# QY-H00/attention-interpolation-diffusion

Measured on AMD Instinct MI355X. Metric: interpolation-frames/sec (50-step), higher is better.
Workload: dtype bf16

## Files before the change

attention-interpolation-diffusion_amd/csrc/aid_gemm.hip:

```cpp
#include "aid_common.hpp"
#include "aid_kernels.hpp"

#include <stdlib.h>
#include <string.h>

#include <type_traits>

namespace aid {

struct TileCoord {
    int p, batch, m0, n0;
};

template <int NB, int MB>
__device__ __forceinline__ void mfma_fence(f32x16 (&acc)[NB][MB]) {
#pragma unroll
    for (int i = 0; i < NB; ++i)
#pragma unroll
        for (int j = 0; j < MB; ++j) asm volatile("" : "+v"(acc[i][j]));
    asm volatile("s_nop 15\n\ts_nop 3" ::: "memory");
#pragma unroll
    for (int i = 0; i < NB; ++i)
#pragma unroll
        for (int j = 0; j < MB; ++j) asm volatile("" : "+v"(acc[i][j]));
// ... 562 lines not shown
                            asm volatile("" : "+v"(t));
                            v[e] = fmaf(lc1[e], t, lr1[im]);
                        }
                    }
#pragma unroll
                    for (int e = 0; e < 4; ++e) v[e] = fmaf(v[e], P.scale, bv[e]);
                    *reinterpret_cast<T4*>(Cs + (wm + im * 32 + l31) * CLD + nl) = cvt4<T>(v);
                }
            }
        __syncthreads();
        const bool vec_ok = (P.ldc % 8 == 0) && ((reinterpret_cast<uintptr_t>(C) & 15) == 0);
        constexpr int CPRW = BN / 8;
#pragma unroll
        for (int it = 0; it < (BM * CPRW) / NTHR; ++it) {
            const int id = tid + it * NTHR;
            const int row = id / CPRW, ch = (id % CPRW) * 8;
            const int m = m0 + row, n = n0 + ch;
            if (m >= P.m || n >= P.n) continue;
            T8 v = *reinterpret_cast<const T8*>(Cs + row * CLD + ch);
            T* dst = C + (int64_t)m * P.ldc + n;
            const T* res = R ? R + (int64_t)m * P.ldc + n : nullptr;
            if (vec_ok && n + 8 <= P.n) {
                if (res) {
                    const bool rvec = (reinterpret_cast<uintptr_t>(R) & 15) == 0;
                    T8 r;
                    if (rvec) {
                        r = *reinterpret_cast<const T8*>(res);
                    } else {
#pragma unroll
                        for (int e = 0; e < 8; ++e) r[e] = res[e];
                    }
                    const f32x8 a = up8<T>(v), b = up8<T>(r);
                    v = cvt8<T>(a + b);
                }
                *reinterpret_cast<T8*>(dst) = v;
            } else {
                const int n4 = (P.n + 3) & ~3;
#pragma unroll
                for (int e = 0; e < 8; ++e) {
                    if (n + e < P.n) dst[e] = res ? (T)((float)v[e] + (float)res[e]) : v[e];
                    else if (n + e < n4) dst[e] = (T)0.f;
                }
            }
        }
    }
};

template <typename T>
struct PingPong : Engine<T, 256, 256, 64, 2, 2, 4> {
    typedef Engine<T, 256, 256, 64, 2, 2, 4> Base;
    typedef typename Vec<T>::v8 T8;
    static constexpr int HALF = 128 * 128;
    static constexpr int STG = 4 * HALF;
    static constexpr size_t SMEM = Base::SMEM;
    using Base::smem; using Base::tid; using Base::lane; using Base::wave; using Base::wm; using Base::wn;
    using Base::l31; using Base::hi; using Base::aoff; using Base::boff; using Base::ax; using Base::bx;
    using Base::acc;
    typedef __amdgpu_buffer_rsrc_t Rsrc;
    int wr;
    Rsrc ra, rb;
    int avo[4], bvo[4];

    static __device__ __forceinline__ int swz(int r) { return (r >> 1) & 7; }

    __device__ __forceinline__ void init(char* smem_) {
        smem = smem_;
        tid = threadIdx.x;
        lane = tid & 63;
        wave = __builtin_amdgcn_readfirstlane(tid >> 6);
        wr = wave >> 2;
        wm = wr * 128;
        wn = (wave & 3) * 64;
        l31 = lane & 31;
        hi = lane >> 5;
#pragma unroll
        for (int e = 0; e < 2; ++e) {
            const int lr = wr * 64 + e * 32 + l31;
            aoff[e] = lr * 128;
            ax[e] = hi ^ swz(lr);
        }
        const int lb = (wave & 3) * 32 + l31;
        boff[0] = 2 * HALF + lb * 128;
        bx[0] = hi ^ swz(lb);
    }

    __device__ __forceinline__ void set_tile(const GemmDesc& P, const T* A, const T* B, int m0, int n0) {
#pragma unroll
        for (int h = 0; h < 2; ++h)
#pragma unroll
            for (int j = 0; j < 2; ++j) {
                const int lrow = 8 * (2 * wave + j) + (lane >> 3);
                const int c = (lane & 7) ^ swz(lrow);
                const int row_a = (lrow >> 6) * 128 + h * 64 + (lrow & 63);
                const int row_b = (lrow >> 5) * 64 + h * 32 + (lrow & 31);
                avo[h * 2 + j] = min(row_a, P.m - 1 - m0) * (P.lda * 2) + c * 16;
                bvo[h * 2 + j] = min(row_b, P.n - 1 - n0) * (P.ldb * 2) + c * 16;
            }
        ra = __builtin_amdgcn_make_buffer_rsrc(const_cast<T*>(A + (int64_t)m0 * P.lda), 0, 0x7fffffff, 0x00020000);
        rb = __builtin_amdgcn_make_buffer_rsrc(const_cast<T*>(B + (int64_t)n0 * P.ldb), 0, 0x7fffffff, 0x00020000);
    }

    __device__ __forceinline__ void set_tile_lr(int m, int n, int lda, int ldb, const T* A, const T* B, int m0, int n0) {
        int ln = lane;
        asm volatile("" : "+v"(ln));
#pragma unroll
        for (int h = 0; h < 2; ++h)
#pragma unroll
            for (int j = 0; j < 2; ++j) {
                const int lrow = 8 * (2 * wave + j) + (ln >> 3);
                const int c = (ln & 7) ^ swz(lrow);
                const int row_a = (lrow >> 6) * 128 + h * 64 + (lrow & 63);
                const int row_b = (lrow >> 5) * 64 + h * 32 + (lrow & 31);
                avo[h * 2 + j] = min(row_a, m - 1 - m0) * (lda * 2) + c * 16;
                bvo[h * 2 + j] = min(row_b, n - 1 - n0) * (ldb * 2) + c * 16;
            }
        ra = __builtin_amdgcn_make_buffer_rsrc(const_cast<T*>(A + (int64_t)m0 * lda), 0, 0x7fffffff, 0x00020000);
        rb = __builtin_amdgcn_make_buffer_rsrc(const_cast<T*>(B + (int64_t)n0 * ldb), 0, 0x7fffffff, 0x00020000);
    }

    static __device__ __forceinline__ float mulg(float a, float g) {
        float t = a * g;
        asm volatile("" : "+v"(t));
        return t;
    }
    __device__ __forceinline__ void scale_rows(const float* __restrict__ gain, int side, int m0, int n0, int M, int N) {
        mfma_fence(acc);
        const bool bym = side == 1;
        const int lim = bym ? M : N;
        float gm[4], gn[2][16];
#pragma unroll
        for (int im = 0; im < 4; ++im) {
            const float g = gain[min(m0 + wm + 32 * im + l31, lim - 1)];
            gm[im] = bym ? g : 1.f;
        }
#pragma unroll
        for (int in = 0; in < 2; ++in)
#pragma unroll
            for (int r = 0; r < 16; ++r) {
                const float g = gain[min(n0 + wn + 32 * in + hi * 4 + 8 * (r >> 2) + (r & 3), lim - 1)];
                gn[in][r] = bym ? 1.f : g;
            }
#pragma unroll
        for (int in = 0; in < 2; ++in)
#pragma unroll
            for (int im = 0; im < 4; ++im)
#pragma unroll
                for (int r = 0; r < 16; ++r) acc[in][im][r] = mulg(mulg(acc[in][im][r], gm[im]), gn[in][r]);
    }

    template <int Q>
    __device__ __forceinline__ void dma_one(int parity, int k0, int j) {
        constexpr bool IS_A = Q >= 2;
        constexpr int H = Q & 1;
        char* dst = smem + parity * STG + (IS_A ? 0 : 2 * HALF) + H * HALF + wave * 2048 + j * 1024;
        __builtin_amdgcn_raw_ptr_buffer_load_lds(IS_A ? ra : rb, (__attribute__((address_space(3))) void*)dst, 16,
                                                 IS_A ? avo[H * 2 + j] : bvo[H * 2 + j], k0 * 2, 0, 0);
    }

    static constexpr int E = 6;
    template <int S>
    __device__ __forceinline__ void issue_first(int kb, int nk) {
        if ((S >> 2) < nk) {
            dma_one<(S & 3)>((S >> 2) & 1, (kb + (S >> 2)) * 64, 0);
            dma_one<(S & 3)>((S >> 2) & 1, (kb + (S >> 2)) * 64, 1);
        }
        if constexpr (S + 1 < E) issue_first<S + 1>(kb, nk);
    }
    template <int P>
    __device__ __forceinline__ void issue(int kt, int kb, int nk, int i) {
        constexpr int S0 = 2 * P + E;
        const int s = S0 + (i >> 1);
        const int t = kt + (s >> 2);
        if (t < nk) {
            if ((S0 & 3) == 2) {
                if (i < 2) dma_one<2>(t & 1, (kb + t) * 64, i & 1);
                else       dma_one<3>(t & 1, (kb + t) * 64, i & 1);
            } else {
                if (i < 2) dma_one<0>(t & 1, (kb + t) * 64, i & 1);
                else       dma_one<1>(t & 1, (kb + t) * 64, i & 1);
            }
        }
    }
    template <int P>
    __device__ __forceinline__ void retire(int kt, int nk) {
        constexpr int NEWEST = 2 * P + E - 1;
        constexpr int NEED = P == 0 ? 3 : 6;
        static_assert(NEWEST >= NEED, "lead too short");
        if (kt + (NEWEST >> 2) < nk) wait_vmcnt<2 * (NEWEST - NEED)>();
        else                         wait_vmcnt<0>();
    }

    __device__ __forceinline__ void read_a(T8 (&fa)[2][4], const char* st, int h) {
#pragma unroll
        for (int e = 0; e < 2; ++e)
#pragma unroll
            for (int ks = 0; ks < 4; ++ks)
                fa[e][ks] = *reinterpret_cast<const T8*>(st + h * HALF + aoff[e] + (((2 * ks) ^ ax[e]) << 4));
    }
    __device__ __forceinline__ void read_b(T8 (&fb)[2][4], const char* st) {
#pragma unroll
        for (int j = 0; j < 2; ++j)
#pragma unroll
            for (int ks = 0; ks < 4; ++ks)
                fb[j][ks] = *reinterpret_cast<const T8*>(st + boff[0] + j * HALF + (((2 * ks) ^ bx[0]) << 4));
    }
    template <int P, bool DMA = true, bool PRIO = false>
    __device__ __forceinline__ void half(const T8 (&fb)[2][4], const T8 (&fa)[2][4], int kt, int kb, int nk) {
        if (PRIO) __builtin_amdgcn_s_setprio(1);
#pragma unroll
        for (int i = 0; i < 16; ++i) {
            const int ks = i >> 2, in = (i >> 1) & 1, e = i & 1;
            acc[in][2 * P + e] = mfma32(fb[in][ks], fa[e][ks], acc[in][2 * P + e]);
            if (DMA && (i == 2 || i == 5 || i == 8 || i == 11)) {
                __builtin_amdgcn_sched_barrier(0);
                issue<P>(kt, kb, nk, (i - 2) / 3);
                __builtin_amdgcn_sched_barrier(0);
            }
        }
        if (PRIO) __builtin_amdgcn_s_setprio(0);
    }
    static __device__ __forceinline__ void slot() {
        __builtin_amdgcn_sched_barrier(0);
        __builtin_amdgcn_s_barrier();
        __builtin_amdgcn_sched_barrier(0);
    }

    template <int Q>
    __device__ __forceinline__ void dma_half(int t, int kb) {
        dma_one<Q>(t & 1, (kb + t) * 64, 0);
        dma_one<Q>(t & 1, (kb + t) * 64, 1);
    }
    template <bool PRIO>
    __device__ __forceinline__ void mac_rd(int kb, int ke) {
        const int nk = ke - kb;
        dma_half<0>(0, kb); dma_half<1>(0, kb); dma_half<2>(0, kb); dma_half<3>(0, kb);
        if (nk > 1) { dma_half<0>(1, kb); dma_half<1>(1, kb); wait_vmcnt<6>(); }
        else        wait_vmcnt<2>();
        slot();
        if (wr == 1) slot();
        T8 fa[2][4], fb[2][4];
        auto body = [&](int kt, auto more1_t, auto more2_t) __attribute__((always_inline)) {
            constexpr bool M1 = decltype(more1_t)::value, M2 = decltype(more2_t)::value;
            const char* st = smem + (kt & 1) * STG;
            read_b(fb, st);
            read_a(fa, st, 0);
            if (M1) { dma_half<2>(kt + 1, kb); dma_half<3>(kt + 1, kb); }
            if (M1) asm volatile("s_waitcnt vmcnt(8) lgkmcnt(0)" ::: "memory");
            else    asm volatile("s_waitcnt vmcnt(0) lgkmcnt(0)" ::: "memory");
            slot();
            half<0, false, PRIO>(fb, fa, kt, kb, nk);
            slot();
            read_a(fa, st, 1);
            if (M2) { dma_half<0>(kt + 2, kb); dma_half<1>(kt + 2, kb); }
            if (M2)      asm volatile("s_waitcnt vmcnt(6) lgkmcnt(0)" ::: "memory");
            else if (M1) asm volatile("s_waitcnt vmcnt(2) lgkmcnt(0)" ::: "memory");
            else         asm volatile("s_waitcnt vmcnt(0) lgkmcnt(0)" ::: "memory");
            slot();
            half<1, false, PRIO>(fb, fa, kt, kb, nk);
            slot();
        };
        const std::true_type Y{};
        const std::false_type N{};
        int kt = 0;
        for (; kt + 2 < nk; ++kt) body(kt, Y, Y);
        if (kt + 1 < nk) { body(kt, Y, N); ++kt; }
        if (kt < nk) body(kt, N, N);
        if (wr == 0) slot();
        wait_vmcnt<0>();
        __syncthreads();
    }

    __device__ __forceinline__ void mac(int kb, int ke) {
        const int nk = ke - kb;
        issue_first<0>(kb, nk);
        if (nk >= 2) wait_vmcnt<2 * (E - 3)>();
        else         wait_vmcnt<0>();
        slot();
        if (wr == 1) slot();
        T8 fa[2][4], fb[2][4];
        for (int kt = 0; kt < nk; ++kt) {
            const char* st = smem + (kt & 1) * STG;
            read_b(fb, st);
            read_a(fa, st, 0);
            retire<0>(kt, nk);
            slot();
            half<0>(fb, fa, kt, kb, nk);
            slot();
            read_a(fa, st, 1);
            retire<1>(kt, nk);
            slot();
            half<1>(fb, fa, kt, kb, nk);
            slot();
        }
        if (wr == 0) slot();
        wait_vmcnt<0>();
        __syncthreads();
    }
};

constexpr int PP_SMALL_NS = 4;
static_assert(Engine<bf16, 128, 128, 64, PP_SMALL_NS, 2, 4>::SMEM <= PingPong<bf16>::SMEM, "small tiles use the big tile's LDS");


template <typename T>
struct PingPongX : PingPong<T> {
    typedef PingPong<T> PP;
    typedef typename Vec<T>::v8 T8;
    typedef typename Vec<T>::v4 T4;
    static constexpr int BMX = 288, XR = 32;
    static constexpr int HALF = PP::HALF;
    static constexpr int STGX = 4 * HALF + XR * 128;
    static constexpr int CLD = 256 + 8;
    static constexpr size_t LNS = (size_t)(BMX + 256) * 2 * sizeof(float);
    static constexpr size_t SMEMX = (size_t)BMX * CLD * 2 + LNS > (size_t)2 * STGX ? (size_t)BMX * CLD * 2 + LNS : (size_t)2 * STGX;
    static_assert(SMEMX <= 160 * 1024, "one workgroup per CU");
    using PP::smem; using PP::tid; using PP::lane; using PP::wave; using PP::wm; using PP::wn; using PP::wr;
    using PP::l31; using PP::hi; using PP::aoff; using PP::boff; using PP::ax; using PP::bx; using PP::acc;
    using PP::ra; using PP::rb; using PP::avo; using PP::bvo;
    f32x16 accx;
    int xoff, xx, xvo;

    __device__ __forceinline__ void init(char* smem_) {
        PP::init(smem_);
        xoff = 4 * HALF + l31 * 128;
        xx = hi ^ PP::swz(l31);
    }
    __device__ __forceinline__ void set_tile(const GemmDesc& P, const T* A, const T* B, int m0, int n0) {
        PP::set_tile(P, A, B, m0, n0);
        const int lrow = 8 * (wave & 3) + (lane >> 3);
        const int c = (lane & 7) ^ PP::swz(lrow);
        xvo = min(256 + lrow, P.m - 1 - m0) * (P.lda * 2) + c * 16;
    }
    __device__ __forceinline__ void zero_acc() {
        PP::zero_acc();
#pragma unroll
        for (int r = 0; r < 16; ++r) accx[r] = 0.f;
    }
    __device__ __forceinline__ void xdma_half(const int Q, int t, int kb) {
        const bool IS_A = Q >= 2;
        const int H = Q & 1;
#pragma unroll
        for (int j = 0; j < 2; ++j) {
            char* dst = smem + (t & 1) * STGX + (IS_A ? 0 : 2 * HALF) + H * HALF + wave * 2048 + j * 1024;
            __builtin_amdgcn_raw_ptr_buffer_load_lds(IS_A ? ra : rb, (__attribute__((address_space(3))) void*)dst, 16,
                                                     IS_A ? avo[H * 2 + j] : bvo[H * 2 + j], (kb + t) * 128, 0, 0);
        }
    }
    __device__ __forceinline__ void dma_strip(int t, int kb) {
        char* dst = smem + (t & 1) * STGX + 4 * HALF + wave * 1024;
        __builtin_amdgcn_raw_ptr_buffer_load_lds(ra, (__attribute__((address_space(3))) void*)dst, 16, xvo, (kb + t) * 128, 0, 0);
    }
    __device__ __forceinline__ void read_x(T8 (&fx)[4], const char* st) {
#pragma unroll
        for (int ks = 0; ks < 4; ++ks) fx[ks] = *reinterpret_cast<const T8*>(st + xoff + (((2 * ks) ^ xx) << 4));
    }
    template <int N>
    __device__ __forceinline__ void wait_rd(bool xw) {
        if (xw) asm volatile("s_waitcnt vmcnt(%0) lgkmcnt(0)" ::"n"(N + 1) : "memory");
        else    asm volatile("s_waitcnt vmcnt(%0) lgkmcnt(0)" ::"n"(N) : "memory");
    }

    template <int WR, bool TR>
    __device__ __forceinline__ void mac_x(int kb, int ke) {
        const int nk = ke - kb;
        const bool xw = wave < 4;
        xdma_half(0, 0, kb); xdma_half(1, 0, kb); xdma_half(2, 0, kb); xdma_half(3, 0, kb);
        if (xw) dma_strip(0, kb);
        if (nk > 1) {
            xdma_half(0, 1, kb); xdma_half(1, 1, kb);
            if (xw) wait_vmcnt<7>(); else wait_vmcnt<6>();
        } else {
            if (xw) wait_vmcnt<3>(); else wait_vmcnt<2>();
        }
        PP::slot();
        if (WR == 1) PP::slot();
        T8 fa[2][4], fb[2][4], fx[4];
        auto body = [&](int kt, auto more1_t, auto more2_t) __attribute__((always_inline)) {
            constexpr bool M1 = decltype(more1_t)::value, M2 = decltype(more2_t)::value;
            const char* st = smem + (kt & 1) * STGX;
            this->read_b(fb, st);
            this->read_a(fa, st, 0);
            if (M1) {
                xdma_half(2, kt + 1, kb); xdma_half(3, kt + 1, kb); if (xw) dma_strip(kt + 1, kb);
                wait_rd<8>(xw);
            } else {
                asm volatile("s_waitcnt vmcnt(0) lgkmcnt(0)" ::: "memory");
            }
            PP::slot();
#pragma unroll
            for (int i = 0; i < 16; ++i) {
                const int ks = i >> 2, in = (i >> 1) & 1, e = i & 1;
                acc[in][e] = TR ? mfma32(fa[e][ks], fb[in][ks], acc[in][e]) : mfma32(fb[in][ks], fa[e][ks], acc[in][e]);
            }
            PP::slot();
            this->read_a(fa, st, 1);
            read_x(fx, st);
            if (M2) {
                xdma_half(0, kt + 2, kb); xdma_half(1, kt + 2, kb);
                wait_rd<6>(xw);
            } else if (M1) {
                wait_rd<2>(xw);
            } else {
                asm volatile("s_waitcnt vmcnt(0) lgkmcnt(0)" ::: "memory");
            }
            PP::slot();
#pragma unroll
            for (int i = 0; i < 16; ++i) {
                const int ks = i >> 2, in = (i >> 1) & 1, e = i & 1;
                acc[in][2 + e] = TR ? mfma32(fa[e][ks], fb[in][ks], acc[in][2 + e]) : mfma32(fb[in][ks], fa[e][ks], acc[in][2 + e]);
                if ((i & 3) == 3)
                    accx = TR ? mfma32(fx[ks], fb[WR][ks], accx) : mfma32(fb[WR][ks], fx[ks], accx);
            }
            PP::slot();
        };
        const std::true_type Y{};
        const std::false_type N{};
        int kt = 0;
        for (; kt + 2 < nk; ++kt) body(kt, Y, Y);
        if (kt + 1 < nk) { body(kt, Y, N); ++kt; }
        if (kt < nk) body(kt, N, N);
        if (WR == 0) PP::slot();
        wait_vmcnt<0>();
        __syncthreads();
    }
    __device__ __forceinline__ void run_tile(const GemmDesc& P, T* C, int batch, int m0, int n0) {
        const int nk = P.k / 64;
        const T* R = P.residual ? reinterpret_cast<const T*>(P.residual) + (int64_t)batch * P.stride_c : nullptr;
        const float* st = P.ln_stats ? P.ln_stats + 2 * (int64_t)batch * P.stride_stats : nullptr;
        if (P.trans_rows) {
            if (wr == 0) { mac_x<0, true>(0, nk); store_tile_t(P, reinterpret_cast<T*>(P.c), m0, n0, P.ln_stats); }
            else         { mac_x<1, true>(0, nk); store_tile_t(P, reinterpret_cast<T*>(P.c), m0, n0, P.ln_stats); }
        } else {
            if (wr == 0) { mac_x<0, false>(0, nk); store_tile(P, C, m0, n0, R, st); }
            else         { mac_x<1, false>(0, nk); store_tile(P, C, m0, n0, R, st); }
        }
    }

    __device__ __forceinline__ void store_tile_t(const GemmDesc& P, T* C, int m0, int n0, const float* stats) {
        constexpr int NTHR = 512, BN = 256, CLDT = BMX + 8;
        static_assert((size_t)BN * CLDT * 2 + LNS <= SMEMX, "transposed C tile fits");
        T* Cs = reinterpret_cast<T*>(smem);
        mfma_fence(acc);
        asm volatile("" : "+v"(accx));
        asm volatile("s_nop 15\n\ts_nop 3" ::: "memory");
        asm volatile("" : "+v"(accx));
        const T* __restrict__ bias = reinterpret_cast<const T*>(P.bias);
        const int side = stats ? P.ln_side : 0;
        float* const lnr = reinterpret_cast<float*>(smem + (size_t)BN * CLDT * 2);
        float* const lnc = lnr + 2 * BMX;
        if (side) {
            for (int i = tid; i < BMX + BN; i += NTHR) {
                const bool isrow = i < BMX;
                const int gi = isrow ? min(m0 + i, P.m - 1) : min(n0 + i - BMX, P.n - 1);
                lnr[2 * i] = isrow ? stats[2 * gi] : P.ln_colsum[gi];
                lnr[2 * i + 1] = isrow ? stats[2 * gi + 1] : P.ln_shift[gi];
            }
            __syncthreads();
        }
        auto stage = [&](const f32x16& a, int rb, int cb) __attribute__((always_inline)) {
            const int col = cb + l31;
            const float bv = (bias && n0 + col < P.n) ? (float)bias[n0 + col] : 0.f;
            float cs = 0.f, sh = 0.f;
            if (side) { cs = lnc[2 * col]; sh = lnc[2 * col + 1]; }
#pragma unroll
            for (int gq = 0; gq < 4; ++gq) {
                const int ml = rb + gq * 8 + hi * 4;
                f32x4 v;
#pragma unroll
                for (int e = 0; e < 4; ++e) v[e] = a[gq * 4 + e];
                if (side) {
                    const f32x4 p0 = *reinterpret_cast<const f32x4*>(lnr + 2 * ml);
                    const f32x4 p1 = *reinterpret_cast<const f32x4*>(lnr + 2 * ml + 4);
                    const float mu[4] = {p0[0], p0[2], p1[0], p1[2]}, rs[4] = {p0[1], p0[3], p1[1], p1[3]};
#pragma unroll
                    for (int e = 0; e < 4; ++e) {
                        float t = fmaf(-mu[e], cs, v[e]);
                        asm volatile("" : "+v"(t));
                        v[e] = fmaf(rs[e], t, sh);
                    }
                }
#pragma unroll
                for (int e = 0; e < 4; ++e) v[e] = fmaf(v[e], P.scale, bv);
                *reinterpret_cast<T4*>(Cs + col * CLDT + ml) = cvt4<T>(v);
            }
        };
#pragma unroll
        for (int in = 0; in < 2; ++in)
#pragma unroll
            for (int im = 0; im < 4; ++im) stage(acc[in][im], wm + im * 32, wn + in * 32);
        stage(accx, 256, wn + wr * 32);
        __syncthreads();
        if (P.trans_rows >= BMX && n0 + BN <= P.n && ((reinterpret_cast<uintptr_t>(C) & 15) == 0)) {
            const int f0 = m0 / P.trans_rows;
            const int next = (f0 + 1) * P.trans_rows - m0;
            constexpr int NPT = (BN * (BMX / 8)) / NTHR;
            T8 v[NPT];
            T* dst[NPT];
#pragma unroll
            for (int it = 0; it < NPT; ++it) {
                const int id = tid + it * NTHR;
                const int col = id / (BMX / 8), chm = (id % (BMX / 8)) * 8;
                v[it] = *reinterpret_cast<const T8*>(Cs + col * CLDT + chm);
                const int f = f0 + (chm >= next ? 1 : 0);
                dst[it] = (m0 + chm < P.m) ? C + (int64_t)f * P.stride_c + (int64_t)(n0 + col) * P.ldc + (m0 + chm - f * P.trans_rows)
                                           : nullptr;
            }
#pragma unroll
            for (int it = 0; it < NPT; ++it)
                if (dst[it]) *reinterpret_cast<T8*>(dst[it]) = v[it];
            return;
        }
        constexpr int CPRW = BMX / 8;
#pragma unroll
        for (int it = 0; it < (BN * CPRW) / NTHR; ++it) {
            const int id = tid + it * NTHR;
            const int col = id / CPRW, ch = (id % CPRW) * 8;
            const int m = m0 + ch, n = n0 + col;
            if (m >= P.m || n >= P.n) continue;
            const int f = m / P.trans_rows, key = m - f * P.trans_rows;
            *reinterpret_cast<T8*>(C + (int64_t)f * P.stride_c + (int64_t)n * P.ldc + key) =
                *reinterpret_cast<const T8*>(Cs + col * CLDT + ch);
        }
    }

    template <int SIDE>
    __device__ __forceinline__ void stage_x_fast(const GemmDesc& P, T* Cs, int n0, const float* lnr, const float* lnc) {
        const T* bias = reinterpret_cast<const T*>(P.bias);
        const float scale = P.scale;
        f32x4 bvx[4];
#pragma unroll
        for (int in = 0; in < 2; ++in) {
            f32x4 bv[4];
            bias_block<T>(bv, bias, n0 + wn + in * 32 + hi * 4);
#pragma unroll
            for (int im = 0; im < 4; ++im)
                stage_block_fast<T, SIDE>(Cs, CLD, acc[in][im], wm + im * 32 + l31, wn + in * 32 + hi * 4, scale, bv, lnr, lnc);
        }
        bias_block<T>(bvx, bias, n0 + wn + wr * 32 + hi * 4);
        stage_block_fast<T, SIDE>(Cs, CLD, accx, 256 + l31, wn + wr * 32 + hi * 4, scale, bvx, lnr, lnc);
    }

    __device__ __forceinline__ void store_tile(const GemmDesc& P, T* C, int m0, int n0, const T* R = nullptr,
                                               const float* stats = nullptr) {
        constexpr int NTHR = 512, BN = 256;
        T* Cs = reinterpret_cast<T*>(smem);
        mfma_fence(acc);
        asm volatile("" : "+v"(accx));
        asm volatile("s_nop 15\n\ts_nop 3" ::: "memory");
        asm volatile("" : "+v"(accx));
        const T* __restrict__ bias = reinterpret_cast<const T*>(P.bias);
        const bool bias_vec = (reinterpret_cast<uintptr_t>(bias) & 7) == 0;
        const int side = stats ? P.ln_side : 0;
        float* const lnr = reinterpret_cast<float*>(smem + (size_t)BMX * CLD * 2);
        float* const lnc = lnr + 2 * BMX;
        if (epilogue_fast_ok<T>(P, C, R, n0, BN)) {
            if (side) {
                for (int i = tid; i < BMX + BN; i += NTHR) {
                    const bool isrow = i < BMX;
                    const int gi = isrow ? min(m0 + i, P.m - 1) : n0 + i - BMX;
                    const bool st = isrow == (side == 1);
                    lnr[2 * i] = st ? stats[2 * gi] : P.ln_colsum[gi];
                    lnr[2 * i + 1] = st ? stats[2 * gi + 1] : P.ln_shift[gi];
                }
                __syncthreads();
            }
            if (side == 0)      stage_x_fast<0>(P, Cs, n0, lnr, lnc);
            else if (side == 1) stage_x_fast<1>(P, Cs, n0, lnr, lnc);
            else                stage_x_fast<2>(P, Cs, n0, lnr, lnc);
            __syncthreads();
            store_rows_fast<T, NTHR, BMX, BN, CLD>(Cs, C, R, m0, n0, P.ldc, min(BMX, P.m - m0), tid);
            return;
        }
        if (side) {
            for (int i = tid; i < BMX + BN; i += NTHR) {
                const bool isrow = i < BMX;
                const int gi = isrow ? min(m0 + i, P.m - 1) : min(n0 + i - BMX, P.n - 1);
                float q0, q1;
                if (isrow == (side == 1)) { q0 = stats[2 * gi]; q1 = stats[2 * gi + 1]; }
                else                      { q0 = P.ln_colsum[gi]; q1 = P.ln_shift[gi]; }
                lnr[2 * i] = q0;
                lnr[2 * i + 1] = q1;
            }
            __syncthreads();
        }
        auto stage = [&](const f32x16& a, int rb, int cb) __attribute__((always_inline)) {
            const int row = rb + l31;
            float lr0 = 0.f, lr1 = 0.f;
            if (side) { lr0 = lnr[2 * row]; lr1 = lnr[2 * row + 1]; }
#pragma unroll
            for (int gq = 0; gq < 4; ++gq) {
                const int nl = cb + gq * 8 + hi * 4;
                f32x4 v;
#pragma unroll
                for (int e = 0; e < 4; ++e) v[e] = a[gq * 4 + e];
                if (side) {
                    const f32x4 p0 = *reinterpret_cast<const f32x4*>(lnc + 2 * nl);
                    const f32x4 p1 = *reinterpret_cast<const f32x4*>(lnc + 2 * nl + 4);
                    const float lc0[4] = {p0[0], p0[2], p1[0], p1[2]}, lc1[4] = {p0[1], p0[3], p1[1], p1[3]};
#pragma unroll
                    for (int e = 0; e < 4; ++e) {
                        float t = side == 1 ? fmaf(-lr0, lc0[e], v[e]) : fmaf(-lc0[e], lr0, v[e]);
                        asm volatile("" : "+v"(t));
                        v[e] = side == 1 ? fmaf(lr1, t, lc1[e]) : fmaf(lc1[e], t, lr1);
                    }
                }
                f32x4 bv = {0.f, 0.f, 0.f, 0.f};
                if (bias) {
                    if (bias_vec && n0 + nl + 4 <= P.n) {
                        bv = up4<T>(*reinterpret_cast<const T4*>(bias + n0 + nl));
                    } else {
#pragma unroll
                        for (int e = 0; e < 4; ++e)
                            if (n0 + nl + e < P.n) bv[e] = (float)bias[n0 + nl + e];
                    }
                }
#pragma unroll
                for (int e = 0; e < 4; ++e) v[e] = fmaf(v[e], P.scale, bv[e]);
                *reinterpret_cast<T4*>(Cs + row * CLD + nl) = cvt4<T>(v);
            }
        };
#pragma unroll
        for (int in = 0; in < 2; ++in)
#pragma unroll
            for (int im = 0; im < 4; ++im) stage(acc[in][im], wm + im * 32, wn + in * 32);
        stage(accx, 256, wn + wr * 32);
        __syncthreads();
        const bool vec_ok = (P.ldc % 8 == 0) && ((reinterpret_cast<uintptr_t>(C) & 15) == 0);
        constexpr int CPRW = BN / 8;
#pragma unroll
        for (int it = 0; it < (BMX * CPRW) / NTHR; ++it) {
            const int id = tid + it * NTHR;
            const int row = id / CPRW, ch = (id % CPRW) * 8;
            const int m = m0 + row, n = n0 + ch;
            if (m >= P.m || n >= P.n) continue;
            T8 v = *reinterpret_cast<const T8*>(Cs + row * CLD + ch);
            T* dst = C + (int64_t)m * P.ldc + n;
            const T* res = R ? R + (int64_t)m * P.ldc + n : nullptr;
            if (vec_ok && n + 8 <= P.n) {
                if (res) {
                    const bool rvec = (reinterpret_cast<uintptr_t>(R) & 15) == 0;
                    T8 r;
                    if (rvec) {
                        r = *reinterpret_cast<const T8*>(res);
                    } else {
#pragma unroll
                        for (int e = 0; e < 8; ++e) r[e] = res[e];
                    }
                    const f32x8 a = up8<T>(v), b = up8<T>(r);
                    v = cvt8<T>(a + b);
                }
                *reinterpret_cast<T8*>(dst) = v;
            } else {
                const int n4 = (P.n + 3) & ~3;
#pragma unroll
                for (int e = 0; e < 8; ++e) {
                    if (n + e < P.n) dst[e] = res ? (T)((float)v[e] + (float)res[e]) : v[e];
                    else if (n + e < n4) dst[e] = (T)0.f;
                }
            }
        }
    }
};
static_assert((288 * 32) % 512 == 0 && (256 * 36) % 512 == 0, "C rows divide over the threads");
static_assert(Engine<bf16, 128, 128, 64, 4, 2, 4>::SMEM <= PingPongX<bf16>::SMEMX, "side tiles use the big tile's LDS");

__device__ __forceinline__ TileCoord locate_side(const GemmSide& sd, int u) {
    int pi = 0;
#pragma unroll
    for (int i = 1; i < 4; ++i)
        if (i < sd.n && u >= sd.tile_start[i]) pi = i;
    const GemmDesc& P = sd.p[pi];
    int rem = u - sd.tile_start[pi];
    const int tiles_n = (P.n + 127) / 128, per_batch = ((P.m + 127) / 128) * tiles_n;
    TileCoord t;
    t.p = pi;
    t.batch = rem / per_batch;
    rem -= t.batch * per_batch;
    t.m0 = (rem / tiles_n) * 128;
    t.n0 = (rem % tiles_n) * 128;
    return t;
}

template <typename T>
__global__ __launch_bounds__(512) void aid_gemm_nt_ppx_kernel(const GemmGroup g, const GemmSide sd) {
    extern __shared__ __attribute__((aligned(16))) char smem_raw[];
    if ((int)blockIdx.x < sd.pad_tiles) {
        const int u = blockIdx.x;
        if (u >= sd.tiles) return;
        const TileCoord t = locate_side(sd, u);
        const GemmDesc& P = sd.p[t.p];
        const int batch = t.batch, m0 = t.m0, n0 = t.n0;
        const T* A = reinterpret_cast<const T*>(P.a) + (int64_t)batch * P.stride_a;
        const T* B = reinterpret_cast<const T*>(P.b) + (int64_t)batch * P.stride_b;
        T* C = reinterpret_cast<T*>(P.c) + (int64_t)batch * P.stride_c;
        Engine<T, 128, 128, 64, 4, 2, 4> e;
        e.init(smem_raw);
        e.set_tile(P, A, B, m0, n0);
        e.zero_acc();
        e.mac(0, P.k / 64);
        e.store_tile(P, C, m0, n0, P.residual ? reinterpret_cast<const T*>(P.residual) + (int64_t)batch * P.stride_c : nullptr,
                     P.ln_stats ? P.ln_stats + 2 * (int64_t)batch * P.stride_stats : nullptr);
        return;
    }
    const int b = blockIdx.x - sd.pad_tiles;
    const TileCoord tc = locate_pos<288, 256>(g, xcd_remap(b, (int)gridDim.x - sd.pad_tiles));
    const GemmDesc& P = g.p[tc.p];
    const T* A = reinterpret_cast<const T*>(P.a) + (int64_t)tc.batch * P.stride_a;
    const T* B = reinterpret_cast<const T*>(P.b) + (int64_t)tc.batch * P.stride_b;
    T* C = reinterpret_cast<T*>(P.c) + (int64_t)tc.batch * P.stride_c;
    PingPongX<T> e;
    e.init(smem_raw);
    e.set_tile(P, A, B, tc.m0, tc.n0);
    e.zero_acc();
    e.run_tile(P, C, tc.batch, tc.m0, tc.n0);
}

template <typename T, int PPV, typename LRT>
__global__ __launch_bounds__(512) void aid_gemm_nt_pp_kernel(const GemmGroup g, const int n_big, const GemmSide sd, const LRT lr) {
    extern __shared__ __attribute__((aligned(16))) char smem_raw[];
    if ((int)blockIdx.x < sd.pad_tiles) {
        const int u = blockIdx.x;
        if (u >= sd.tiles) return;
        const TileCoord t = locate_side(sd, u);
        const GemmDesc& P = sd.p[t.p];
        const int batch = t.batch, m0 = t.m0, n0 = t.n0;
        const T* A = reinterpret_cast<const T*>(P.a) + (int64_t)batch * P.stride_a;
        const T* B = reinterpret_cast<const T*>(P.b) + (int64_t)batch * P.stride_b;
        T* C = reinterpret_cast<T*>(P.c) + (int64_t)batch * P.stride_c;
        Engine<T, 128, 128, 64, PP_SMALL_NS, 2, 4> e;
        e.init(smem_raw);
        e.set_tile(P, A, B, m0, n0);
        e.zero_acc();
        e.mac(0, P.k / 64);
        e.store_tile(P, C, m0, n0, P.residual ? reinterpret_cast<const T*>(P.residual) + (int64_t)batch * P.stride_c : nullptr,
                     P.ln_stats ? P.ln_stats + 2 * (int64_t)batch * P.stride_stats : nullptr);
        return;
    }
    const int b = blockIdx.x - sd.pad_tiles;
    if (b < n_big) {
        const TileCoord tc = locate_pos<256, 256>(g, xcd_remap(b, n_big));
        const GemmDesc& P = g.p[tc.p];
        const T* A = reinterpret_cast<const T*>(P.a) + (int64_t)tc.batch * P.stride_a;
        const T* B = reinterpret_cast<const T*>(P.b) + (int64_t)tc.batch * P.stride_b;
        T* C = reinterpret_cast<T*>(P.c) + (int64_t)tc.batch * P.stride_c;
        PingPong<T> e;
        e.init(smem_raw);
        e.set_tile(P, A, B, tc.m0, tc.n0);
        e.zero_acc();
        if (PPV == 1)      e.template mac_rd<false>(0, P.k / 64);
        else if (PPV == 2) e.template mac_rd<true>(0, P.k / 64);
        else               e.mac(0, P.k / 64);
        if constexpr (std::is_same<LRT, GemmLR>::value) {
            const GemmLRDesc& L = lr.p[tc.p];
            if (L.k > 0) {
                e.set_tile_lr(P.m, P.n, L.lda, L.ldb, reinterpret_cast<const T*>(L.a) + (int64_t)tc.batch * L.stride_a,
                              reinterpret_cast<const T*>(L.b) + (int64_t)tc.batch * L.stride_b, tc.m0, tc.n0);
                if (PPV == 1)      e.template mac_rd<false>(0, L.k / 64);
                else if (PPV == 2) e.template mac_rd<true>(0, L.k / 64);
                else               e.mac(0, L.k / 64);
            }
            if (L.row_scale) e.scale_rows(L.row_scale, L.side, tc.m0, tc.n0, P.m, P.n);
        }
        e.store_tile(P, C, tc.m0, tc.n0, P.residual ? reinterpret_cast<const T*>(P.residual) + (int64_t)tc.batch * P.stride_c : nullptr,
                     P.ln_stats ? P.ln_stats + 2 * (int64_t)tc.batch * P.stride_stats : nullptr);
    } else {
        const int u = b - n_big;
        const int n_rest = ((int)gridDim.x - sd.pad_tiles - n_big) >> 2;
        const int quad = u / n_rest, t = u - quad * n_rest;
        TileCoord tc = locate_pos<256, 256>(g, n_big + xcd_remap(t, n_rest));
        const GemmDesc& P = g.p[tc.p];
        tc.m0 += (quad >> 1) * 128;
        tc.n0 += (quad & 1) * 128;
        if (tc.m0 >= P.m || tc.n0 >= P.n) return;
        const T* A = reinterpret_cast<const T*>(P.a) + (int64_t)tc.batch * P.stride_a;
        const T* B = reinterpret_cast<const T*>(P.b) + (int64_t)tc.batch * P.stride_b;
        T* C = reinterpret_cast<T*>(P.c) + (int64_t)tc.batch * P.stride_c;
        Engine<T, 128, 128, 64, PP_SMALL_NS, 2, 4> e;
        e.init(smem_raw);
        e.set_tile(P, A, B, tc.m0, tc.n0);
        e.zero_acc();
        e.mac(0, P.k / 64);
        if constexpr (std::is_same<LRT, GemmLR>::value) {
            const GemmLRDesc& L = lr.p[tc.p];
            if (L.k > 0) {
                e.set_tile_lr(P.m, P.n, L.lda, L.ldb, reinterpret_cast<const T*>(L.a) + (int64_t)tc.batch * L.stride_a,
                              reinterpret_cast<const T*>(L.b) + (int64_t)tc.batch * L.stride_b, tc.m0, tc.n0);
                e.mac(0, L.k / 64);
            }
            if (L.row_scale) {
                mfma_fence(e.acc);
                lr_row_scale(e.acc, L.row_scale, L.side, tc.m0 + e.wm + e.l31, tc.n0 + e.wn + e.hi * 4, P.m, P.n);
            }
        }
        e.store_tile(P, C, tc.m0, tc.n0, P.residual ? reinterpret_cast<const T*>(P.residual) + (int64_t)tc.batch * P.stride_c : nullptr,
                     P.ln_stats ? P.ln_stats + 2 * (int64_t)tc.batch * P.stride_stats : nullptr);
    }
}

template <typename T, int BM, int BN, int BK, int NS, int WM, int WN, typename LRT>
__global__ __launch_bounds__(WM * WN * 64) void aid_gemm_nt_pipe_kernel(const GemmGroup g, const LRT lr) {
    extern __shared__ __attribute__((aligned(16))) char smem_raw[];
    const TileCoord tc = locate_tile<BM, BN>(g, blockIdx.x, gridDim.x);
    const GemmDesc& P = g.p[tc.p];
    const T* A = reinterpret_cast<const T*>(P.a) + (int64_t)tc.batch * P.stride_a;
    const T* B = reinterpret_cast<const T*>(P.b) + (int64_t)tc.batch * P.stride_b;
    T* C = reinterpret_cast<T*>(P.c) + (int64_t)tc.batch * P.stride_c;
    Engine<T, BM, BN, BK, NS, WM, WN> e;
    e.init(smem_raw);
    e.set_tile(P, A, B, tc.m0, tc.n0);
    e.zero_acc();
    e.mac(0, P.k / BK);
    if constexpr (std::is_same<LRT, GemmLR>::value) {
        const GemmLRDesc& L = lr.p[tc.p];
        if (L.k > 0) {
            e.set_tile_lr(P.m, P.n, L.lda, L.ldb, reinterpret_cast<const T*>(L.a) + (int64_t)tc.batch * L.stride_a,
                          reinterpret_cast<const T*>(L.b) + (int64_t)tc.batch * L.stride_b, tc.m0, tc.n0);
            e.mac(0, L.k / BK);
        }
        if (L.row_scale) {
            mfma_fence(e.acc);
            lr_row_scale(e.acc, L.row_scale, L.side, tc.m0 + e.wm + e.l31, tc.n0 + e.wn + e.hi * 4, P.m, P.n);
        }
    }
    e.store_tile(P, C, tc.m0, tc.n0, P.residual ? reinterpret_cast<const T*>(P.residual) + (int64_t)tc.batch * P.stride_c : nullptr,
                     P.ln_stats ? P.ln_stats + 2 * (int64_t)tc.batch * P.stride_stats : nullptr);
}

static int tiles_of(const GemmDesc& d, int bm, int bn) { return ((d.m + bm - 1) / bm) * ((d.n + bn - 1) / bn) * d.batch; }

static int count_tiles(const GemmGroup& g, int bm, int bn) {
    int tiles = 0;
    for (int i = 0; i < g.n_problems; ++i) tiles += tiles_of(g.p[i], bm, bn);
    return tiles;
}

int fill_tile_start(GemmGroup& g, int bm, int bn) {
    int tiles = 0;
    for (int i = 0; i < g.n_problems; ++i) {
        g.tile_start[i] = tiles;
        tiles += tiles_of(g.p[i], bm, bn);
    }
    for (int i = g.n_problems; i <= AID_GEMM_MAX_PROBLEMS; ++i) g.tile_start[i] = tiles;
    return tiles;
}

template <typename K, typename LRT>
static hipError_t launch_with_smem(K kernel, size_t smem, PerDevice<int>& attr_set, GemmGroup& g, int bm, int bn, hipStream_t stream,
                                   int threads, const LRT& lr) {
    const int tiles = fill_tile_start(g, bm, bn);
    if (tiles <= 0) return hipSuccess;
    const hipError_t e = set_max_dynamic_lds(attr_set, 0, reinterpret_cast<const void*>(kernel), smem);
    if (e != hipSuccess) return e;
    hipLaunchKernelGGL(kernel, dim3(tiles), dim3(threads), smem, stream, g, lr);
    return hipGetLastError();
}

template <typename T, typename LRT>
static hipError_t launch_edge(GemmGroup& g, hipStream_t stream, const LRT& lr) {
    static PerDevice<int> attr_set;
    return launch_with_smem(aid_gemm_nt_kernel<T, LRT>, (size_t)2 * (GBM + GBN) * GLD * sizeof(T), attr_set, g, GBM, GBN, stream, GTHREADS,
                            lr);
}

template <typename T, int NS, typename LRT>
static hipError_t launch_pipe(GemmGroup& g, hipStream_t stream, const LRT& lr) {
    static PerDevice<int> attr_set;
    return launch_with_smem(aid_gemm_nt_pipe_kernel<T, 128, 128, 64, NS, 2, 4, LRT>, Engine<T, 128, 128, 64, NS, 2, 4>::SMEM, attr_set, g,
                            128, 128, stream, 512, lr);
}

template <typename T, int PPV, typename LRT>
static hipError_t launch_pp_v(GemmGroup& g, hipStream_t stream, int n_big, int n_small, const GemmSide& sd, const LRT& lr) {
    static PerDevice<int> attr_set;
    if (fill_tile_start(g, 256, 256) <= 0) return hipSuccess;
    const hipError_t e = set_max_dynamic_lds(attr_set, 0, reinterpret_cast<const void*>(aid_gemm_nt_pp_kernel<T, PPV, LRT>), PingPong<T>::SMEM);
    if (e != hipSuccess) return e;
    hipLaunchKernelGGL((aid_gemm_nt_pp_kernel<T, PPV, LRT>), dim3(sd.pad_tiles + n_big + n_small), dim3(512), PingPong<T>::SMEM, stream,
                       g, n_big, sd, lr);
    return hipGetLastError();
}
template <typename T, typename LRT>
static hipError_t launch_pp(GemmGroup& g, hipStream_t stream, int n_big, int n_small, const GemmSide& sd, const LRT& lr) {
    switch (tune(TUNE_GEMM_PP)) {
        case 0:  return launch_pp_v<T, 0>(g, stream, n_big, n_small, sd, lr);
        case 2:  return launch_pp_v<T, 2>(g, stream, n_big, n_small, sd, lr);
        default: return launch_pp_v<T, 1>(g, stream, n_big, n_small, sd, lr);
    }
}

template <typename T>
static hipError_t launch_ppx(GemmGroup& g, hipStream_t stream, const GemmSide& sd) {
    static PerDevice<int> attr_set;
    const int tiles = fill_tile_start(g, 288, 256);
    if (tiles <= 0) return hipSuccess;
    const hipError_t e = set_max_dynamic_lds(attr_set, 0, reinterpret_cast<const void*>(aid_gemm_nt_ppx_kernel<T>), PingPongX<T>::SMEMX);
    if (e != hipSuccess) return e;
    hipLaunchKernelGGL(aid_gemm_nt_ppx_kernel<T>, dim3(sd.pad_tiles + tiles), dim3(512), PingPongX<T>::SMEMX, stream, g, sd);
    return hipGetLastError();
}

int device_cu_count() {
    static PerDevice<int> cus;
    int* n = cus.slot();
    if (!n) return 0;
    if (*n == 0) {
        int dev = 0;
        hipDeviceProp_t pr;
        if (hipGetDevice(&dev) != hipSuccess || hipGetDeviceProperties(&pr, dev) != hipSuccess) return 0;
        *n = pr.multiProcessorCount;
    }
    return *n;
}

struct PpSplit {
    int n_big, n_small;
    double rounds;
};
static PpSplit split_pp(int tiles, int ncu, int nk) {
    PpSplit s;
    const int full = tiles / ncu, rest = tiles % ncu;
    s.n_big = tiles;
    s.n_small = 0;
    s.rounds = full + (rest ? 1 : 0);
    if (full > 0 && rest > 0 && rest <= ncu / 2 && ncu % 8 == 0) {
        s.n_big = full * ncu;
        s.n_small = 4 * rest;
        s.rounds = full + ((4 * rest + ncu - 1) / ncu) * (2.0 + 0.6 * nk) / (6.0 + 1.62 * nk);
    }
// ... 237 lines not shown
```

Before: 3.973.

## Switch PingPongX GEMM inner loop from 32x32 to 16x16x32 MFMA tiles

```diff
diff --git a/attention-interpolation-diffusion_amd/csrc/aid_gemm.hip b/attention-interpolation-diffusion_amd/csrc/aid_gemm.hip
--- a/attention-interpolation-diffusion_amd/csrc/aid_gemm.hip
+++ b/attention-interpolation-diffusion_amd/csrc/aid_gemm.hip
@@ -888,6 +888,13 @@
 static_assert(Engine<bf16, 128, 128, 64, PP_SMALL_NS, 2, 4>::SMEM <= PingPong<bf16>::SMEM, "small tiles use the big tile's LDS");
 
 
+__device__ __forceinline__ f32x4 mfma16(const Vec<f16>::v8& a, const Vec<f16>::v8& b, const f32x4& c) {
+    return __builtin_amdgcn_mfma_f32_16x16x32_f16(a, b, c, 0, 0, 0);
+}
+__device__ __forceinline__ f32x4 mfma16(const Vec<bf16>::v8& a, const Vec<bf16>::v8& b, const f32x4& c) {
+    return __builtin_amdgcn_mfma_f32_16x16x32_bf16(a, b, c, 0, 0, 0);
+}
+
 template <typename T>
 struct PingPongX : PingPong<T> {
     typedef PingPong<T> PP;
@@ -903,13 +910,17 @@
     using PP::smem; using PP::tid; using PP::lane; using PP::wave; using PP::wm; using PP::wn; using PP::wr;
     using PP::l31; using PP::hi; using PP::aoff; using PP::boff; using PP::ax; using PP::bx; using PP::acc;
     using PP::ra; using PP::rb; using PP::avo; using PP::bvo;
-    f32x16 accx;
-    int xoff, xx, xvo;
+    f32x4 c[2][4][2][2], cx[2][2];
+    int l15, kg, a16, b16, x16, cxr, xvo;
 
     __device__ __forceinline__ void init(char* smem_) {
         PP::init(smem_);
-        xoff = 4 * HALF + l31 * 128;
-        xx = hi ^ PP::swz(l31);
+        l15 = lane & 15;
+        kg = lane >> 4;
+        a16 = (wr * 64 + l15) * 128;
+        b16 = 2 * HALF + ((wave & 3) * 32 + l15) * 128;
+        x16 = 4 * HALF + l15 * 128;
+        cxr = kg ^ PP::swz(l15);
     }
     __device__ __forceinline__ void set_tile(const GemmDesc& P, const T* A, const T* B, int m0, int n0) {
         PP::set_tile(P, A, B, m0, n0);
@@ -918,9 +929,21 @@
         xvo = min(256 + lrow, P.m - 1 - m0) * (P.lda * 2) + c * 16;
     }
     __device__ __forceinline__ void zero_acc() {
-        PP::zero_acc();
-#pragma unroll
-        for (int r = 0; r < 16; ++r) accx[r] = 0.f;
+#pragma unroll
+        for (int i = 0; i < 32; ++i) (&c[0][0][0][0])[i] = f32x4{0.f, 0.f, 0.f, 0.f};
+#pragma unroll
+        for (int i = 0; i < 4; ++i) (&cx[0][0])[i] = f32x4{0.f, 0.f, 0.f, 0.f};
+    }
+    __device__ __forceinline__ void fence() {
+#pragma unroll
+        for (int i = 0; i < 32; ++i) asm volatile("" : "+v"((&c[0][0][0][0])[i]));
+#pragma unroll
+        for (int i = 0; i < 4; ++i) asm volatile("" : "+v"((&cx[0][0])[i]));
+        asm volatile("s_nop 15\n\ts_nop 3" ::: "memory");
+#pragma unroll
+        for (int i = 0; i < 32; ++i) asm volatile("" : "+v"((&c[0][0][0][0])[i]));
+#pragma unroll
+        for (int i = 0; i < 4; ++i) asm volatile("" : "+v"((&cx[0][0])[i]));
     }
     __device__ __forceinline__ void xdma_half(const int Q, int t, int kb) {
         const bool IS_A = Q >= 2;
@@ -936,9 +959,25 @@
         char* dst = smem + (t & 1) * STGX + 4 * HALF + wave * 1024;
         __builtin_amdgcn_raw_ptr_buffer_load_lds(ra, (__attribute__((address_space(3))) void*)dst, 16, xvo, (kb + t) * 128, 0, 0);
     }
-    __device__ __forceinline__ void read_x(T8 (&fx)[4], const char* st) {
-#pragma unroll
-        for (int ks = 0; ks < 4; ++ks) fx[ks] = *reinterpret_cast<const T8*>(st + xoff + (((2 * ks) ^ xx) << 4));
+    __device__ __forceinline__ void read_a16(T8 (&fa)[4][2], const char* st, int h) {
+#pragma unroll
+        for (int eb = 0; eb < 4; ++eb)
+#pragma unroll
+            for (int j = 0; j < 2; ++j)
+                fa[eb][j] = *reinterpret_cast<const T8*>(st + h * HALF + a16 + eb * 2048 + (((4 * j) ^ cxr) << 4));
+    }
+    __device__ __forceinline__ void read_b16(T8 (&fb)[4][2], const char* st) {
+#pragma unroll
+        for (int bb = 0; bb < 4; ++bb)
+#pragma unroll
+            for (int j = 0; j < 2; ++j)
+                fb[bb][j] = *reinterpret_cast<const T8*>(st + b16 + (bb >> 1) * HALF + (bb & 1) * 2048 + (((4 * j) ^ cxr) << 4));
+    }
+    __device__ __forceinline__ void read_x16(T8 (&fx)[2][2], const char* st) {
+#pragma unroll
+        for (int sm = 0; sm < 2; ++sm)
+#pragma unroll
+            for (int j = 0; j < 2; ++j) fx[sm][j] = *reinterpret_cast<const T8*>(st + x16 + sm * 2048 + (((4 * j) ^ cxr) << 4));
     }
     template <int N>
     __device__ __forceinline__ void wait_rd(bool xw) {
@@ -960,12 +999,12 @@
         }
         PP::slot();
         if (WR == 1) PP::slot();
-        T8 fa[2][4], fb[2][4], fx[4];
+        T8 fa[4][2], fb[4][2], fx[2][2];
         auto body = [&](int kt, auto more1_t, auto more2_t) __attribute__((always_inline)) {
             constexpr bool M1 = decltype(more1_t)::value, M2 = decltype(more2_t)::value;
             const char* st = smem + (kt & 1) * STGX;
-            this->read_b(fb, st);
-            this->read_a(fa, st, 0);
+            read_b16(fb, st);
+            read_a16(fa, st, 0);
             if (M1) {
                 xdma_half(2, kt + 1, kb); xdma_half(3, kt + 1, kb); if (xw) dma_strip(kt + 1, kb);
                 wait_rd<8>(xw);
@@ -974,13 +1013,14 @@
             }
             PP::slot();
 #pragma unroll
-            for (int i = 0; i < 16; ++i) {
-                const int ks = i >> 2, in = (i >> 1) & 1, e = i & 1;
-                acc[in][e] = TR ? mfma32(fa[e][ks], fb[in][ks], acc[in][e]) : mfma32(fb[in][ks], fa[e][ks], acc[in][e]);
+            for (int i = 0; i < 32; ++i) {
+                const int j = i >> 4, bb = (i >> 2) & 3, eb = i & 3;
+                f32x4& d = c[bb >> 1][eb >> 1][bb & 1][eb & 1];
+                d = TR ? mfma16(fa[eb][j], fb[bb][j], d) : mfma16(fb[bb][j], fa[eb][j], d);
             }
             PP::slot();
-            this->read_a(fa, st, 1);
-            read_x(fx, st);
+            read_a16(fa, st, 1);
+            read_x16(fx, st);
             if (M2) {
                 xdma_half(0, kt + 2, kb); xdma_half(1, kt + 2, kb);
                 wait_rd<6>(xw);
@@ -991,11 +1031,14 @@
             }
             PP::slot();
 #pragma unroll
-            for (int i = 0; i < 16; ++i) {
-                const int ks = i >> 2, in = (i >> 1) & 1, e = i & 1;
-                acc[in][2 + e] = TR ? mfma32(fa[e][ks], fb[in][ks], acc[in][2 + e]) : mfma32(fb[in][ks], fa[e][ks], acc[in][2 + e]);
-                if ((i & 3) == 3)
-                    accx = TR ? mfma32(fx[ks], fb[WR][ks], accx) : mfma32(fb[WR][ks], fx[ks], accx);
+            for (int i = 0; i < 32; ++i) {
+                const int j = i >> 4, bb = (i >> 2) & 3, eb = i & 3;
+                f32x4& d = c[bb >> 1][2 + (eb >> 1)][bb & 1][eb & 1];
+                d = TR ? mfma16(fa[eb][j], fb[bb][j], d) : mfma16(fb[bb][j], fa[eb][j], d);
+                if ((i & 3) == 3) {
+                    const int s = i >> 2, js = s >> 2, sn = (s >> 1) & 1, sm = s & 1;
+                    cx[sn][sm] = TR ? mfma16(fx[sm][js], fb[2 * WR + sn][js], cx[sn][sm]) : mfma16(fb[2 * WR + sn][js], fx[sm][js], cx[sn][sm]);
+                }
             }
             PP::slot();
         };
@@ -1026,10 +1069,7 @@
         constexpr int NTHR = 512, BN = 256, CLDT = BMX + 8;
         static_assert((size_t)BN * CLDT * 2 + LNS <= SMEMX, "transposed C tile fits");
         T* Cs = reinterpret_cast<T*>(smem);
-        mfma_fence(acc);
-        asm volatile("" : "+v"(accx));
-        asm volatile("s_nop 15\n\ts_nop 3" ::: "memory");
-        asm volatile("" : "+v"(accx));
+        fence();
         const T* __restrict__ bias = reinterpret_cast<const T*>(P.bias);
         const int side = stats ? P.ln_side : 0;
         float* const lnr = reinterpret_cast<float*>(smem + (size_t)BN * CLDT * 2);
@@ -1043,38 +1083,48 @@
             }
             __syncthreads();
         }
-        auto stage = [&](const f32x16& a, int rb, int cb) __attribute__((always_inline)) {
-            const int col = cb + l31;
-            const float bv = (bias && n0 + col < P.n) ? (float)bias[n0 + col] : 0.f;
-            float cs = 0.f, sh = 0.f;
+        auto stage = [&](const f32x4& a, int ml, int col, float bv, float cs, float sh) __attribute__((always_inline)) {
+            f32x4 v = a;
+            if (side) {
+                const f32x4 p0 = *reinterpret_cast<const f32x4*>(lnr + 2 * ml);
+                const f32x4 p1 = *reinterpret_cast<const f32x4*>(lnr + 2 * ml + 4);
+                const float mu[4] = {p0[0], p0[2], p1[0], p1[2]}, rs[4] = {p0[1], p0[3], p1[1], p1[3]};
+#pragma unroll
+                for (int e = 0; e < 4; ++e) {
+                    float t = fmaf(-mu[e], cs, v[e]);
+                    asm volatile("" : "+v"(t));
+                    v[e] = fmaf(rs[e], t, sh);
+                }
+            }
+#pragma unroll
+            for (int e = 0; e < 4; ++e) v[e] = fmaf(v[e], P.scale, bv);
+            *reinterpret_cast<T4*>(Cs + col * CLDT + ml) = cvt4<T>(v);
+        };
+        auto column = [&](int col, float& bv, float& cs, float& sh) __attribute__((always_inline)) {
+            bv = (bias && n0 + col < P.n) ? (float)bias[n0 + col] : 0.f;
+            cs = 0.f; sh = 0.f;
             if (side) { cs = lnc[2 * col]; sh = lnc[2 * col + 1]; }
-#pragma unroll
-            for (int gq = 0; gq < 4; ++gq) {
-                const int ml = rb + gq * 8 + hi * 4;
-                f32x4 v;
-#pragma unroll
-                for (int e = 0; e < 4; ++e) v[e] = a[gq * 4 + e];
-                if (side) {
-                    const f32x4 p0 = *reinterpret_cast<const f32x4*>(lnr + 2 * ml);
-                    const f32x4 p1 = *reinterpret_cast<const f32x4*>(lnr + 2 * ml + 4);
-                    const float mu[4] = {p0[0], p0[2], p1[0], p1[2]}, rs[4] = {p0[1], p0[3], p1[1], p1[3]};
-#pragma unroll
-                    for (int e = 0; e < 4; ++e) {
-                        float t = fmaf(-mu[e], cs, v[e]);
-                        asm volatile("" : "+v"(t));
-                        v[e] = fmaf(rs[e], t, sh);
-                    }
-                }
-#pragma unroll
-                for (int e = 0; e < 4; ++e) v[e] = fmaf(v[e], P.scale, bv);
-                *reinterpret_cast<T4*>(Cs + col * CLDT + ml) = cvt4<T>(v);
-            }
         };
 #pragma unroll
         for (int in = 0; in < 2; ++in)
 #pragma unroll
-            for (int im = 0; im < 4; ++im) stage(acc[in][im], wm + im * 32, wn + in * 32);
-        stage(accx, 256, wn + wr * 32);
+            for (int sn = 0; sn < 2; ++sn) {
+                const int col = wn + in * 32 + sn * 16 + l15;
+                float bv, cs, sh;
+                column(col, bv, cs, sh);
+#pragma unroll
+                for (int im = 0; im < 4; ++im)
+#pragma unroll
+                    for (int sm = 0; sm < 2; ++sm) stage(c[in][im][sn][sm], wm + im * 32 + sm * 16 + kg * 4, col, bv, cs, sh);
+            }
+#pragma unroll
+        for (int sn = 0; sn < 2; ++sn) {
+            const int col = wn + wr * 32 + sn * 16 + l15;
+            float bv, cs, sh;
+            column(col, bv, cs, sh);
+#pragma unroll
+            for (int sm = 0; sm < 2; ++sm) stage(cx[sn][sm], 256 + sm * 16 + kg * 4, col, bv, cs, sh);
+        }
         __syncthreads();
         if (P.trans_rows >= BMX && n0 + BN <= P.n && ((reinterpret_cast<uintptr_t>(C) & 15) == 0)) {
             const int f0 = m0 / P.trans_rows;
@@ -1113,27 +1163,63 @@
     __device__ __forceinline__ void stage_x_fast(const GemmDesc& P, T* Cs, int n0, const float* lnr, const float* lnc) {
         const T* bias = reinterpret_cast<const T*>(P.bias);
         const float scale = P.scale;
-        f32x4 bvx[4];
-#pragma unroll
-        for (int in = 0; in < 2; ++in) {
-            f32x4 bv[4];
-            bias_block<T>(bv, bias, n0 + wn + in * 32 + hi * 4);
-#pragma unroll
-            for (int im = 0; im < 4; ++im)
-                stage_block_fast<T, SIDE>(Cs, CLD, acc[in][im], wm + im * 32 + l31, wn + in * 32 + hi * 4, scale, bv, lnr, lnc);
-        }
-        bias_block<T>(bvx, bias, n0 + wn + wr * 32 + hi * 4);
-        stage_block_fast<T, SIDE>(Cs, CLD, accx, 256 + l31, wn + wr * 32 + hi * 4, scale, bvx, lnr, lnc);
+        auto stage = [&](const f32x4& a, int row, int nl, const f32x4& bv, const float (&c0)[4], const float (&c1)[4]) __attribute__((always_inline)) {
+            f32x4 v = a;
+            if (SIDE) {
+                const float lr0 = lnr[2 * row], lr1 = lnr[2 * row + 1];
+#pragma unroll
+                for (int e = 0; e < 4; ++e) {
+                    float t = SIDE == 1 ? fmaf(-lr0, c0[e], v[e]) : fmaf(-c0[e], lr0, v[e]);
+                    asm volatile("" : "+v"(t));
+                    v[e] = SIDE == 1 ? fmaf(lr1, t, c1[e]) : fmaf(c1[e], t, lr1);
+                }
+            }
+#pragma unroll
+            for (int e = 0; e < 4; ++e) {
+                float t = fmaf(v[e], scale, bv[e]);
+                asm volatile("" : "+v"(t));
+                v[e] = t;
+            }
+            *reinterpret_cast<T4*>(Cs + row * CLD + nl) = cvt4<T>(v);
+        };
+        auto columns = [&](int nl, f32x4& bv, float (&c0)[4], float (&c1)[4]) __attribute__((always_inline)) {
+            bv = bias ? up4<T>(*reinterpret_cast<const T4*>(bias + n0 + nl)) : f32x4{0.f, 0.f, 0.f, 0.f};
+            if (SIDE) {
+                const f32x4 p0 = *reinterpret_cast<const f32x4*>(lnc + 2 * nl);
+                const f32x4 p1 = *reinterpret_cast<const f32x4*>(lnc + 2 * nl + 4);
+                c0[0] = p0[0]; c0[1] = p0[2]; c0[2] = p1[0]; c0[3] = p1[2];
+                c1[0] = p0[1]; c1[1] = p0[3]; c1[2] = p1[1]; c1[3] = p1[3];
+            }
+        };
+#pragma unroll
+        for (int in = 0; in < 2; ++in)
+#pragma unroll
+            for (int sn = 0; sn < 2; ++sn) {
+                const int nl = wn + in * 32 + sn * 16 + kg * 4;
+                f32x4 bv;
+                float c0[4] = {0.f, 0.f, 0.f, 0.f}, c1[4] = {0.f, 0.f, 0.f, 0.f};
+                columns(nl, bv, c0, c1);
+#pragma unroll
+                for (int im = 0; im < 4; ++im)
+#pragma unroll
+                    for (int sm = 0; sm < 2; ++sm) stage(c[in][im][sn][sm], wm + im * 32 + sm * 16 + l15, nl, bv, c0, c1);
+            }
+#pragma unroll
+        for (int sn = 0; sn < 2; ++sn) {
+            const int nl = wn + wr * 32 + sn * 16 + kg * 4;
+            f32x4 bv;
+            float c0[4] = {0.f, 0.f, 0.f, 0.f}, c1[4] = {0.f, 0.f, 0.f, 0.f};
+            columns(nl, bv, c0, c1);
+#pragma unroll
+            for (int sm = 0; sm < 2; ++sm) stage(cx[sn][sm], 256 + sm * 16 + l15, nl, bv, c0, c1);
+        }
     }
 
     __device__ __forceinline__ void store_tile(const GemmDesc& P, T* C, int m0, int n0, const T* R = nullptr,
                                                const float* stats = nullptr) {
         constexpr int NTHR = 512, BN = 256;
         T* Cs = reinterpret_cast<T*>(smem);
-        mfma_fence(acc);
-        asm volatile("" : "+v"(accx));
-        asm volatile("s_nop 15\n\ts_nop 3" ::: "memory");
-        asm volatile("" : "+v"(accx));
+        fence();
         const T* __restrict__ bias = reinterpret_cast<const T*>(P.bias);
         const bool bias_vec = (reinterpret_cast<uintptr_t>(bias) & 7) == 0;
         const int side = stats ? P.ln_side : 0;
@@ -1169,47 +1255,49 @@
             }
             __syncthreads();
         }
-        auto stage = [&](const f32x16& a, int rb, int cb) __attribute__((always_inline)) {
-            const int row = rb + l31;
+        auto stage = [&](const f32x4& a, int rb, int cb) __attribute__((always_inline)) {
+            const int row = rb + l15;
             float lr0 = 0.f, lr1 = 0.f;
             if (side) { lr0 = lnr[2 * row]; lr1 = lnr[2 * row + 1]; }
-#pragma unroll
-            for (int gq = 0; gq < 4; ++gq) {
-                const int nl = cb + gq * 8 + hi * 4;
-                f32x4 v;
-#pragma unroll
-                for (int e = 0; e < 4; ++e) v[e] = a[gq * 4 + e];
-                if (side) {
-                    const f32x4 p0 = *reinterpret_cast<const f32x4*>(lnc + 2 * nl);
-                    const f32x4 p1 = *reinterpret_cast<const f32x4*>(lnc + 2 * nl + 4);
-                    const float lc0[4] = {p0[0], p0[2], p1[0], p1[2]}, lc1[4] = {p0[1], p0[3], p1[1], p1[3]};
-#pragma unroll
-                    for (int e = 0; e < 4; ++e) {
-                        float t = side == 1 ? fmaf(-lr0, lc0[e], v[e]) : fmaf(-lc0[e], lr0, v[e]);
-                        asm volatile("" : "+v"(t));
-                        v[e] = side == 1 ? fmaf(lr1, t, lc1[e]) : fmaf(lc1[e], t, lr1);
-                    }
+            const int nl = cb + kg * 4;
+            f32x4 v = a;
+            if (side) {
+                const f32x4 p0 = *reinterpret_cast<const f32x4*>(lnc + 2 * nl);
+                const f32x4 p1 = *reinterpret_cast<const f32x4*>(lnc + 2 * nl + 4);
+                const float lc0[4] = {p0[0], p0[2], p1[0], p1[2]}, lc1[4] = {p0[1], p0[3], p1[1], p1[3]};
+#pragma unroll
+                for (int e = 0; e < 4; ++e) {
+                    float t = side == 1 ? fmaf(-lr0, lc0[e], v[e]) : fmaf(-lc0[e], lr0, v[e]);
+                    asm volatile("" : "+v"(t));
+                    v[e] = side == 1 ? fmaf(lr1, t, lc1[e]) : fmaf(lc1[e], t, lr1);
                 }
-                f32x4 bv = {0.f, 0.f, 0.f, 0.f};
-                if (bias) {
-                    if (bias_vec && n0 + nl + 4 <= P.n) {
-                        bv = up4<T>(*reinterpret_cast<const T4*>(bias + n0 + nl));
-                    } else {
-#pragma unroll
-                        for (int e = 0; e < 4; ++e)
-                            if (n0 + nl + e < P.n) bv[e] = (float)bias[n0 + nl + e];
-                    }
+            }
+            f32x4 bv = {0.f, 0.f, 0.f, 0.f};
+            if (bias) {
+                if (bias_vec && n0 + nl + 4 <= P.n) {
+                    bv = up4<T>(*reinterpret_cast<const T4*>(bias + n0 + nl));
+                } else {
+#pragma unroll
+                    for (int e = 0; e < 4; ++e)
+                        if (n0 + nl + e < P.n) bv[e] = (float)bias[n0 + nl + e];
                 }
-#pragma unroll
-                for (int e = 0; e < 4; ++e) v[e] = fmaf(v[e], P.scale, bv[e]);
-                *reinterpret_cast<T4*>(Cs + row * CLD + nl) = cvt4<T>(v);
-            }
+            }
+#pragma unroll
+            for (int e = 0; e < 4; ++e) v[e] = fmaf(v[e], P.scale, bv[e]);
+            *reinterpret_cast<T4*>(Cs + row * CLD + nl) = cvt4<T>(v);
         };
 #pragma unroll
         for (int in = 0; in < 2; ++in)
 #pragma unroll
-            for (int im = 0; im < 4; ++im) stage(acc[in][im], wm + im * 32, wn + in * 32);
-        stage(accx, 256, wn + wr * 32);
+            for (int im = 0; im < 4; ++im)
+#pragma unroll
+                for (int sn = 0; sn < 2; ++sn)
+#pragma unroll
+                    for (int sm = 0; sm < 2; ++sm) stage(c[in][im][sn][sm], wm + im * 32 + sm * 16, wn + in * 32 + sn * 16);
+#pragma unroll
+        for (int sn = 0; sn < 2; ++sn)
+#pragma unroll
+            for (int sm = 0; sm < 2; ++sm) stage(cx[sn][sm], 256 + sm * 16, wn + wr * 32 + sn * 16);
         __syncthreads();
         const bool vec_ok = (P.ldc % 8 == 0) && ((reinterpret_cast<uintptr_t>(C) & 15) == 0);
         constexpr int CPRW = BN / 8;
```

Result: faster. 4.104 (median of 6 runs) (+3.3%).
